# Jason9339/Wavelet-Noise-in-ray-tracing

Hardware: AMD Instinct MI355X
Metric: Mnoise-samples/sec (3D wavelet, octave=4) (higher is better)
Workload: dtype f32; 1 GPU; 512^3 dense 3D WNoise grid, tile=128, octave=4 (configs[1]); tile=128, seed=12345, octave=4, device=AMD Radeon Graphics (gfx950:sramecc+:xnack-)

## Files before the change

wavelet-noise-in-ray-tracing_amd/csrc/wn_wavelet_multiband.hip:

```cpp
#include "wn_internal.hpp"

#include <algorithm>
#include <cmath>
#include <type_traits>

namespace {

using wn::GridArgs;

typedef float v4f __attribute__((ext_vector_type(4)));
typedef float v2f __attribute__((ext_vector_type(2)));

constexpr int kMaxNB = 5;
constexpr int kWW = 8, kPW = 4, kSW = 4;
constexpr int kWaves = kWW + kPW + kSW;
constexpr int kPasses = 2 * kPW;
constexpr int kBX = 512, kBY = 8, kBZ = 8;
constexpr int kRing = 4;
constexpr int kSlotZ = 8, kSlotX = 16;
constexpr int kMaxK = 5;
constexpr int kRRow = kPasses * 64;
constexpr int kRPlane = kBY * kRRow;
constexpr int kRingFloats = kRing * kBY * kBX;
constexpr int kBoxFloats = 6144;
constexpr int kDmaPlanes = kMaxNB;
constexpr int kDmaLanded = kBZ - 2;

struct MbBand {
    float oscale;
    float factor;
    int first_pass;
    int K;
    int box_off;
    int rowlen;
};

struct MbArgs {
    const float *coef;
    float *out;
    int n, nmask;
    GridArgs g;
    float inv_den;
    int nbx, nby, nbz;
    int all_full;
    MbBand band[kMaxNB];
    int pass_band[kPasses];
};

__device__ __forceinline__ float readlane_f(float v, int l)
{
    return __int_as_float(__builtin_amdgcn_readlane(__float_as_int(v), l));
}

template <int NB>
__global__ __launch_bounds__(64 * kWaves) void grid3d_mbp_kernel(const MbArgs a)
{
    extern __shared__ __attribute__((aligned(16))) float lds[];
    __shared__ __attribute__((aligned(16))) float s_box[kBoxFloats];
    __shared__ int s_mid[3][NB][32];
    __shared__ float s_w[3][NB][kSlotX][3];
    __shared__ float s_oscale[NB];
    __shared__ __attribute__((aligned(16))) float s_wy[NB][kMaxK][kBY];
    __shared__ float s_wz[NB][64];
    __shared__ int s_prep[NB][4];
    __shared__ int s_bandc[NB][4];

    const int tid = threadIdx.x, lane = tid & 63;
    const int wave = __builtin_amdgcn_readfirstlane(tid >> 6);
    const bool is_window = wave < kWW, is_collapse = wave >= kWW && wave < kWW + kPW;
    const GridArgs &g = a.g;
    float *const ring = lds + 2 * kRPlane;

    const int nyz = a.nby * a.nbz;
    const long long total = (long long)a.nbx * nyz;
    const int item0 = (int)(total * blockIdx.x / gridDim.x), item1 = (int)(total * (blockIdx.x + 1) / gridDim.x);
    const int nb = item1 - item0;
    if (nb <= 0) return;
    const int G = nb * kBZ;

    struct Brick { int bx, by, bz; };
    auto brick_of = [&](int item) {
        Brick k;
        k.bx = item / nyz;
        k.by = (item - k.bx * nyz) / a.nbz;
        k.bz = item - k.bx * nyz - k.by * a.nbz;
        return k;
    };
    auto advance = [&](Brick &k) {
        if (++k.bz == a.nbz) { k.bz = 0; ++k.by; }
        if (k.by == a.nby) { k.by = 0; ++k.bx; }
    };

    auto fill_tables = [&](int buf, const Brick &k) {
        int tt = tid;
        asm volatile("" : "+v"(tt));
        const int b = tt >> 5, slot = tt & 31;
        if (b < NB && slot < kSlotX + 2) {
            int idx;
            if (slot < kSlotZ) idx = min(k.by * kBY + slot, g.ny - 1);
            else if (slot < kSlotX) idx = g.z0 + min(k.bz * kBZ + slot - kSlotZ, g.nz - 1);
            else idx = (slot == kSlotX) ? k.bx * kBX : min(k.bx * kBX + kBX - 1, g.nx - 1);
            const float c = wn::lattice_coord_fast(idx, (float)g.den, a.inv_den, g.base_range, s_oscale[b], g.post_scale);
            int m;
            float w0, w1, w2;
            wn::bspline(c, m, w0, w1, w2);
            s_mid[buf][b][slot] = m;
            if (slot < kSlotX) {
                s_w[buf][b][slot][0] = w0;
                s_w[buf][b][slot][1] = w1;
                s_w[buf][b][slot][2] = w2;
            }
        }
    };
    auto sgpr = [](int v) { return __builtin_amdgcn_readfirstlane(v); };
    auto fresh_rows = [&](int b, int K, int tA, int tB, bool same_column) {
        const int d = sgpr(s_mid[tB][b][kSlotZ]) - sgpr(s_mid[tA][b][kSlotZ]);
        return (same_column && d >= 0 && d <= 2) ? d : K;
    };

    auto derive_tables = [&](int b, int tA, int tB, bool same_column, bool first) {
        const int l = lane;
        {
            const int K = s_bandc[b][0];
            const int kz0 = s_mid[tB][b][kSlotZ] - 1;
            const int kzm = (K == 4) ? (kz0 & 3) : ((kz0 + 20 * 65536) % 5);
            {
                const int zi = l >> 3, j = l & 7;
                int t0 = kzm + (s_mid[tB][b][kSlotZ + zi] - s_mid[tB][b][kSlotZ]);
                t0 -= (t0 >= K) ? K : 0;
                const float w0 = s_w[tB][b][kSlotZ + zi][0], w1 = s_w[tB][b][kSlotZ + zi][1], w2 = s_w[tB][b][kSlotZ + zi][2];
                s_wz[b][l] = j == 0 ? w0 : j == 1 ? w1 : j == 2 ? w2 : __int_as_float(t0);
            }
            if (l < kMaxK * kBY) {
                const int j = l >> 3, yi = l & 7;
                const int dd = j - (s_mid[tB][b][yi] - s_mid[tB][b][0]);
                const float w0 = s_w[tB][b][yi][0], w1 = s_w[tB][b][yi][1], w2 = s_w[tB][b][yi][2];
                float f = a.band[0].factor;
#pragma unroll
                for (int bb = 1; bb < NB; ++bb) f = (b == bb) ? a.band[bb].factor : f;
                s_wy[b][j][yi] = ((unsigned)dd <= 2u ? (dd == 0 ? w0 : dd == 1 ? w1 : w2) : 0.0f) * f;
            }
            if (l == 0) {
                const int dz = s_mid[tB][b][kSlotZ] - s_mid[tA][b][kSlotZ];
                s_prep[b][0] = kzm;
                s_prep[b][1] = (!first && same_column && dz >= 0 && dz <= 2) ? dz : K;
                s_prep[b][2] = (s_mid[tB][b][kSlotX] - 1) & 3;
            }
        }
    };

    Brick cur = brick_of(item0), nxt = cur;
    advance(nxt);
    Brick nxt2 = nxt;
    advance(nxt2);
    if (tid < NB) {
        int K = a.band[0].K, box_off = a.band[0].box_off, rowlen = a.band[0].rowlen, fp = a.band[0].first_pass;
#pragma unroll
        for (int bb = 1; bb < NB; ++bb) {
            K = (tid == bb) ? a.band[bb].K : K;
            box_off = (tid == bb) ? a.band[bb].box_off : box_off;
            rowlen = (tid == bb) ? a.band[bb].rowlen : rowlen;
            fp = (tid == bb) ? a.band[bb].first_pass : fp;
        }
        s_bandc[tid][0] = K;
        s_bandc[tid][1] = box_off;
        s_bandc[tid][2] = rowlen;
        s_bandc[tid][3] = fp;
        float os = a.band[0].oscale;
#pragma unroll
        for (int bb = 1; bb < NB; ++bb) os = (tid == bb) ? a.band[bb].oscale : os;
        s_oscale[tid] = os;
    }
    __syncthreads();
    fill_tables(0, cur);
    if (nb > 1) fill_tables(1, nxt);
    __syncthreads();
    int tb = 0, t = 0;
    auto next_brick = [&]() {
        cur = nxt;
        nxt = nxt2;
        advance(nxt2);
        tb = (tb == 2) ? 0 : tb + 1;
        ++t;
    };

    if (is_collapse) {
        struct Pass {
            int id, band, col0, box_off, rowlen;
            float factor;
        };
        Pass ps[2];
        int pk[2];
#pragma unroll
        for (int i = 0; i < 2; ++i) {
            Pass &P = ps[i];
            P.id = (wave - kWW) + kPW * i;
            P.band = sgpr(a.pass_band[P.id]);
            const int bb0 = max(P.band, 0);
            pk[i] = P.band >= 0 ? sgpr(s_bandc[bb0][0]) : 0;
            P.box_off = sgpr(s_bandc[bb0][1]);
            P.rowlen = sgpr(s_bandc[bb0][2]);
            P.col0 = 64 * (P.id - sgpr(s_bandc[bb0][3]));
            float f = a.band[0].factor;
#pragma unroll
            for (int bb = 1; bb < NB; ++bb) f = (bb0 == bb) ? a.band[bb].factor : f;
            P.factor = __int_as_float(sgpr(__float_as_int(f)));
        }
        auto prep_brick = [&](const Pass &P, auto &yc, float &wzv, auto kc) {
            constexpr int K = decltype(kc)::value;
            if constexpr (K > 0) {
                const int kzm = sgpr(s_prep[P.band][0]), d = sgpr(s_prep[P.band][1]);
                wzv = s_wz[P.band][lane];
                const float *img = s_box + P.box_off + min(sgpr(s_prep[P.band][2]) + P.col0 + lane, P.rowlen - 1);
#pragma unroll
                for (int sl = 0; sl < K; ++sl) {
                    const int tau = (sl - kzm + K) % K;
                    if (tau >= K - d) {
                        const float *row = img + (tau - (K - d)) * K * P.rowlen;
#pragma unroll
                        for (int j = 0; j < K; ++j) {
                            const float cj = row[j * P.rowlen];
                            const v2f c2 = {cj, cj};
#pragma unroll
                            for (int h = 0; h < 2; ++h) {
                                const v4f w4 = *reinterpret_cast<const v4f *>(&s_wy[P.band][j][4 * h]);
                                const v2f wlo = {w4.x, w4.y}, whi = {w4.z, w4.w};
                                yc[2 * h][sl] = (j == 0) ? wlo * c2 : __builtin_elementwise_fma(wlo, c2, yc[2 * h][sl]);
                                yc[2 * h + 1][sl] = (j == 0) ? whi * c2 : __builtin_elementwise_fma(whi, c2, yc[2 * h + 1][sl]);
                            }
                        }
                    }
                }
            }
        };
        auto p1_slice = [&](float *Rw, int zi, const auto &yc, float wzv, auto kc) {
            constexpr int K = decltype(kc)::value;
            if constexpr (K > 0) {
                const float w0 = readlane_f(wzv, zi * 8), w1 = readlane_f(wzv, zi * 8 + 1), w2 = readlane_f(wzv, zi * 8 + 2);
                const int t0 = __builtin_amdgcn_readlane(__float_as_int(wzv), zi * 8 + 3);
                auto taps = [&](auto tc) {
                    constexpr int T0 = decltype(tc)::value, T1 = (T0 + 1) % K, T2 = (T0 + 2) % K;
#pragma unroll
                    for (int p2 = 0; p2 < kBY / 2; ++p2) {
                        v2f v = v2f{w0, w0} * yc[p2][T0];
                        v = __builtin_elementwise_fma(v2f{w1, w1}, yc[p2][T1], v);
                        v = __builtin_elementwise_fma(v2f{w2, w2}, yc[p2][T2], v);
                        Rw[(2 * p2) * kRRow] = v.x;
                        Rw[(2 * p2 + 1) * kRRow] = v.y;
                    }
                };
                using std::integral_constant;
                if (t0 == 0) taps(integral_constant<int, 0>{});
                else if (t0 == 1) taps(integral_constant<int, 1>{});
                else if (t0 == 2) taps(integral_constant<int, 2>{});
                else if (t0 == 3 || K == 4) taps(integral_constant<int, 3>{});
                else taps(integral_constant<int, K - 1>{});
            }
        };
        auto collapse_role = [&](auto k0c, auto k1c) {
            constexpr int K0 = decltype(k0c)::value, K1 = decltype(k1c)::value;
            v2f yc0[kBY / 2][K0 > 0 ? K0 : 1], yc1[kBY / 2][K1 > 0 ? K1 : 1];
            float wzv0 = 0.0f, wzv1 = 0.0f;
            float *const Rw0 = lds + 64 * ps[0].id + lane, *const Rw1 = lds + 64 * ps[1].id + lane;
            wn::lds_barrier();
            prep_brick(ps[0], yc0, wzv0, k0c);
            prep_brick(ps[1], yc1, wzv1, k1c);
            p1_slice(Rw0, 0, yc0, wzv0, k0c);
            p1_slice(Rw1, 0, yc1, wzv1, k1c);
            wn::lds_barrier();
            for (int gp = 0; gp < G + 2; ++gp) {
                const int zi = gp & (kBZ - 1);
                if (gp < G) {
                    if (gp + 1 < G) {
                        if (zi == kBZ - 1) {
                            prep_brick(ps[0], yc0, wzv0, k0c);
                            prep_brick(ps[1], yc1, wzv1, k1c);
                        }
                        const int rs = ((gp + 1) & 1) * kRPlane;
                        p1_slice(Rw0 + rs, (gp + 1) & (kBZ - 1), yc0, wzv0, k0c);
                        p1_slice(Rw1 + rs, (gp + 1) & (kBZ - 1), yc1, wzv1, k1c);
                    }
                    if (zi == kBZ - 1) next_brick();
                }
                wn::lds_barrier();
            }
        };
        using std::integral_constant;
        const int k0 = pk[0], k1 = pk[1];
        if (k0 == 4 && k1 == 4) collapse_role(integral_constant<int, 4>{}, integral_constant<int, 4>{});
        else if (k0 == 4 && k1 == 5) collapse_role(integral_constant<int, 4>{}, integral_constant<int, 5>{});
        else if (k0 == 5 && k1 == 4) collapse_role(integral_constant<int, 5>{}, integral_constant<int, 4>{});
        else if (k0 == 5 && k1 == 5) collapse_role(integral_constant<int, 5>{}, integral_constant<int, 5>{});
        else if (k0 == 4) collapse_role(integral_constant<int, 4>{}, integral_constant<int, 0>{});
        else if (k0 == 5) collapse_role(integral_constant<int, 5>{}, integral_constant<int, 0>{});
        else collapse_role(integral_constant<int, 0>{}, integral_constant<int, 0>{});
    } else if (is_window) {
        const int xw = (wave >> 2) & 1, wr = wave & 3;
        float ww[NB][4][4];
        int wbase[NB];
        auto x_weights = [&](int tbuf, int bx) {
            const float den = (float)g.den;
            const int x0 = bx * kBX + xw * 256 + lane * 4;
            float xbase[4];
#pragma unroll
            for (int q = 0; q < 4; ++q) {
                const float xi = (float)min(x0 + q, g.nx - 1);
                xbase[q] = ((a.inv_den != 0.0f) ? xi * a.inv_den : xi / den) * g.base_range;
            }
#pragma unroll
            for (int b = 0; b < NB; ++b) {
                int m[4];
                float w[4][3];
#pragma unroll
                for (int q = 0; q < 4; ++q) {
                    float cc = xbase[q] * a.band[b].oscale;
                    cc = cc * g.post_scale;
                    wn::bspline(cc, m[q], w[q][0], w[q][1], w[q][2]);
                }
                wbase[b] = 64 * a.band[b].first_pass + m[0] - s_mid[tbuf][b][kSlotX];
#pragma unroll
                for (int q = 0; q < 4; ++q) {
                    const bool up = m[q] != m[0];
                    ww[b][q][0] = up ? 0.0f : w[q][0];
                    ww[b][q][1] = up ? w[q][0] : w[q][1];
                    ww[b][q][2] = up ? w[q][1] : w[q][2];
                    ww[b][q][3] = up ? w[q][2] : 0.0f;
                }
            }
        };
        auto phaseC = [&](int rslot, int ringslot) {
            float acc[2][4];
            const float *Rp = lds + rslot * kRPlane + wr * kRRow;
#pragma unroll
            for (int b = 0; b < NB; ++b) {
                float v[2][4];
#pragma unroll
                for (int h = 0; h < 2; ++h)
#pragma unroll
                    for (int i = 0; i < 4; ++i) v[h][i] = Rp[h * 4 * kRRow + wbase[b] + i];
#pragma unroll
                for (int h = 0; h < 2; ++h)
#pragma unroll
                    for (int q = 0; q < 4; ++q) {
                        float s = (b == 0) ? ww[b][q][0] * v[h][0] : __builtin_fmaf(ww[b][q][0], v[h][0], acc[h][q]);
                        s = __builtin_fmaf(ww[b][q][1], v[h][1], s);
                        s = __builtin_fmaf(ww[b][q][2], v[h][2], s);
                        s = __builtin_fmaf(ww[b][q][3], v[h][3], s);
                        acc[h][q] = s;
                    }
            }
#pragma unroll
            for (int h = 0; h < 2; ++h)
                *reinterpret_cast<v4f *>(ring + (ringslot * kBY + wr + 4 * h) * kBX + xw * 256 + lane * 4) =
                    v4f{acc[h][0], acc[h][1], acc[h][2], acc[h][3]};
        };

        x_weights(0, cur.bx);
        wn::lds_barrier();
        wn::lds_barrier();
        for (int gp = 0; gp < G + 2; ++gp) {
            const int zi = gp & (kBZ - 1);
            if (gp < G) {
                phaseC(gp & 1, gp & (kRing - 1));
                if (zi == kBZ - 1) {
                    const int tb1 = (tb == 2) ? 0 : tb + 1, tb2 = (tb1 == 2) ? 0 : tb1 + 1;
                    if (t + 2 < nb) fill_tables(tb2, nxt2);
                    if (t + 1 < nb && nxt.bx != cur.bx) x_weights(tb1, nxt.bx);
                    next_brick();
                }
            }
            wn::lds_barrier();
        }
    } else {
        const int sw = wave - (kWW + kPW);
        int bK[NB], bBox[NB], bRow[NB];
#pragma unroll
        for (int b = 0; b < NB; ++b) {
            bK[b] = sgpr(s_bandc[b][0]);
            bBox[b] = sgpr(s_bandc[b][1]);
            bRow[b] = sgpr(s_bandc[b][2]);
        }
        auto request_band = [&](auto bc, int tA, int tB, bool same_column, bool first) {
            constexpr int b = decltype(bc)::value;
            if constexpr (b < NB) {
                const int K = bK[b];
                const int d = first ? K : fresh_rows(b, K, tA, tB, same_column);
                const int jy0 = sgpr(s_mid[tB][b][0]) - 1, kz0 = sgpr(s_mid[tB][b][kSlotZ]) - 1 + (K - d);
                const int r = min(lane, K * K - 1);
                const int f = (K == 4) ? (r >> 2) : ((r * 13) >> 6);
                const int j = r - f * K;
                const int rowoff = (((kz0 + f) & a.nmask) * a.n + ((jy0 + j) & a.nmask)) * a.n;
                const int ix0 = (sgpr(s_mid[tB][b][kSlotX]) - 1) & ~3;
                const unsigned voff = (unsigned)((ix0 + 4 * lane) & a.nmask) * 4u;
                for (int rr = sw; rr < d * K; rr += kSW) {
                    const char *rowp = reinterpret_cast<const char *>(a.coef + __builtin_amdgcn_readlane(rowoff, rr));
                    if (4 * lane < bRow[b])
                        __builtin_amdgcn_global_load_lds((const __attribute__((address_space(1))) void *)(rowp + voff),
                                                         (__attribute__((address_space(3))) void *)&s_box[bBox[b] + rr * bRow[b]],
                                                         16, 0, 0);
                }
            }
        };
        Brick sb = cur;
        const size_t plane_stride = (size_t)g.ny * g.nx;
        float *orow = nullptr;
        auto brick_pointer = [&]() {
            orow = a.out + ((size_t)(sb.bz * kBZ) * g.ny + sb.by * kBY + 2 * sw) * g.nx + sb.bx * kBX + lane * 4;
        };
        brick_pointer();
        auto store_plane = [&](int p) {
            const int zi = p & (kBZ - 1), ringslot = p & (kRing - 1);
            const float *src = ring + (ringslot * kBY + 2 * sw) * kBX + lane * 4;
            v4f v[4];
#pragma unroll
            for (int q = 0; q < 4; ++q) v[q] = *reinterpret_cast<const v4f *>(src + (q >> 1) * kBX + (q & 1) * 256);
            if (a.all_full) {
#pragma unroll
                for (int q = 0; q < 4; ++q) *reinterpret_cast<v4f *>(orow + (size_t)(q >> 1) * g.nx + (q & 1) * 256) = v[q];
            } else {
                const int z = sb.bz * kBZ + zi;
#pragma unroll
                for (int q = 0; q < 4; ++q) {
                    const int row = 2 * sw + (q >> 1), xh = q & 1;
                    const int y = sb.by * kBY + row, x = sb.bx * kBX + xh * 256 + lane * 4;
                    if (y < g.ny && z < g.nz && x + 3 < g.nx)
                        *reinterpret_cast<v4f *>(orow + (size_t)(q >> 1) * g.nx + (q & 1) * 256) = v[q];
                }
            }
            orow += plane_stride;
            if (zi == kBZ - 1) {
                advance(sb);
                brick_pointer();
            }
        };

        using std::integral_constant;
        request_band(integral_constant<int, 0>{}, 0, 0, false, true);
        request_band(integral_constant<int, 1>{}, 0, 0, false, true);
        request_band(integral_constant<int, 2>{}, 0, 0, false, true);
        request_band(integral_constant<int, 3>{}, 0, 0, false, true);
        request_band(integral_constant<int, 4>{}, 0, 0, false, true);
        for (int b = sw; b < NB; b += kSW) derive_tables(b, 0, 0, false, true);
        asm volatile("s_waitcnt vmcnt(0)" ::: "memory");
        wn::lds_barrier();
        wn::lds_barrier();
        for (int gp = 0; gp < G + 2; ++gp) {
            const int zi = gp & (kBZ - 1);
            if (gp >= 2) store_plane(gp - 2);
            if (gp < G) {
                if (zi < NB && t + 1 < nb) {
                    const int tb1 = (tb == 2) ? 0 : tb + 1;
                    const bool same = nxt.bx == cur.bx && nxt.by == cur.by;
                    if (zi == 0) request_band(integral_constant<int, 0>{}, tb, tb1, same, false);
                    else if (zi == 1) request_band(integral_constant<int, 1>{}, tb, tb1, same, false);
                    else if (zi == 2) request_band(integral_constant<int, 2>{}, tb, tb1, same, false);
                    else if (zi == 3) request_band(integral_constant<int, 3>{}, tb, tb1, same, false);
                    else request_band(integral_constant<int, 4>{}, tb, tb1, same, false);
                }
                if (zi == kBZ - 2 && t + 1 < nb)
                    for (int b = sw; b < NB; b += kSW)
                        derive_tables(b, tb, (tb == 2) ? 0 : tb + 1, nxt.bx == cur.bx && nxt.by == cur.by, false);
                if (zi == kDmaLanded) {
                    if (a.all_full) asm volatile("s_waitcnt vmcnt(%0)" ::"n"(4 * (kDmaLanded - kDmaPlanes + 1)) : "memory");
                    else asm volatile("s_waitcnt vmcnt(0)" ::: "memory");
                }
                if (zi == kBZ - 1) next_brick();
            }
            wn::lds_barrier();
        }
    }
}

template <int NB>
bool launch_mbp(const MbArgs &a, size_t lds, long long bricks, hipStream_t s)
{
    const void *fn = reinterpret_cast<const void *>(&grid3d_mbp_kernel<NB>);
    if (!wn::ensure_dynamic_lds(fn, wn::current_device(), lds)) return false;
    const int cus = wn::device_compute_units(wn::current_device());
    const int grid = (int)std::min<long long>(bricks, cus);
    hipLaunchKernelGGL((grid3d_mbp_kernel<NB>), dim3(grid), dim3(64 * kWaves), lds, s, a);
    return true;
}

}

namespace wn {

int multiband_try(const wn_tile *tile, const GridArgs &g, int nbands, const float *oscale, const float *weights,
                  float out_div, float *out_dev, hipStream_t stream, int min_bricks_per_cu)
{
    if (nbands < 1 || nbands > kMaxNB || tile->n == 0 || wn::pow2_mask(tile->n) < 0) return kDeclined;
    if (g.nx <= 256 || !vec4_ok(out_dev, g.nx) || g.ny <= 0 || g.nz <= 0 || g.z_const_mode || g.z0 < 0) return kDeclined;
    MbArgs a{};
    int passes = 0, box_off = 0;
    for (int w = 0; w < kPasses; ++w) a.pass_band[w] = -1;
    for (int b = 0; b < nbands; ++b) {
        LatticeStep ls;
        if (!lattice_step(g, oscale[b], false, false, 0.0, &ls) || !ls.two_mids()) return kDeclined;
        const int K = (int)std::max<long long>(4, std::max(ls.extent(kBY), ls.extent(kBZ)));
        if (K > kMaxK) return kDeclined;
        const int ex = (int)ls.extent(kBX) + 1;
        const int np = (ex + 63) / 64;
        if (passes + np > kPasses) return kDeclined;
        a.band[b].first_pass = passes;
        for (int p = 0; p < np; ++p) a.pass_band[passes++] = b;
        a.band[b].oscale = oscale[b];
        a.band[b].factor = (float)((double)(weights ? weights[b] : 1.0f) * (double)g.out_scale / (double)out_div);
        a.band[b].K = K;
        a.band[b].rowlen = (ex + 3 + 3) & ~3;
        if (a.band[b].rowlen > 256) return kDeclined;
        a.band[b].box_off = box_off;
        box_off += K * K * a.band[b].rowlen;
    }
    if (box_off > kBoxFloats) return kDeclined;
    const size_t lds = (size_t)(2 * kRPlane + kRingFloats) * sizeof(float);
    a.coef = tile->dev;
    a.out = out_dev;
    a.n = tile->n;
    a.nmask = wn::pow2_mask(tile->n);
    a.g = g;
    a.inv_den = wn::inv_den_of(g.den);
    a.nbx = (g.nx + kBX - 1) / kBX;
    a.nby = (g.ny + kBY - 1) / kBY;
    a.nbz = (g.nz + kBZ - 1) / kBZ;
    a.all_full = (g.nx % kBX == 0 && g.ny % kBY == 0 && g.nz % kBZ == 0) ? 1 : 0;
    const long long bricks = (long long)a.nbx * a.nby * a.nbz;
    if (bricks > 0x7fffffffLL / kBZ) return kDeclined;
    if (bricks < (long long)min_bricks_per_cu * wn::device_compute_units(wn::current_device())) return kDeclined;
    if ((long long)a.nbx * kBX * 10 > (long long)g.nx * 11) return kDeclined;
    bool ok;
    switch (nbands) {
    case 1: ok = launch_mbp<1>(a, lds, bricks, stream); break;
    case 2: ok = launch_mbp<2>(a, lds, bricks, stream); break;
    case 3: ok = launch_mbp<3>(a, lds, bricks, stream); break;
    case 4: ok = launch_mbp<4>(a, lds, bricks, stream); break;
    default: ok = launch_mbp<5>(a, lds, bricks, stream); break;
    }
    if (!ok) return kDeclined;
    WN_LAUNCH_CHECK("grid3d_mbp_kernel");
    return WN_OK;
}

}
```

Before: 1.419 million Msamples/s.

## Overlap prologue coefficient DMA with table fill and trim derive_tables work

The store waves now compute the first brick's lattice midpoints themselves and issue the initial coefficient row DMAs right away, while the other waves fill both table buffers in parallel. This replaces the two __syncthreads and the serialized first request_band calls. derive_tables now handles two bands per wave across lane halves with a compact z-weight layout, and recomputes the y-weight table only when the brick column changes. This mainly shortens per-block prologue latency and per-brick derive cost, at the price of more intricate lane mapping and duplicated midpoint computation.

```diff
diff --git a/wavelet-noise-in-ray-tracing_amd/csrc/wn_wavelet_multiband.hip b/wavelet-noise-in-ray-tracing_amd/csrc/wn_wavelet_multiband.hip
--- a/wavelet-noise-in-ray-tracing_amd/csrc/wn_wavelet_multiband.hip
+++ b/wavelet-noise-in-ray-tracing_amd/csrc/wn_wavelet_multiband.hip
@@ -91,16 +91,24 @@
         if (k.by == a.nby) { k.by = 0; ++k.bx; }
     };
 
-    auto fill_tables = [&](int buf, const Brick &k) {
-        int tt = tid;
+    auto oscale_of = [&](int b) {
+        float os = a.band[0].oscale;
+#pragma unroll
+        for (int bb = 1; bb < NB; ++bb) os = (b == bb) ? a.band[bb].oscale : os;
+        return os;
+    };
+    auto fill_tables = [&](int buf, const Brick &k, int tt, auto from_args) {
         asm volatile("" : "+v"(tt));
         const int b = tt >> 5, slot = tt & 31;
-        if (b < NB && slot < kSlotX + 2) {
+        if (tt >= 0 && b < NB && slot < kSlotX + 2) {
             int idx;
             if (slot < kSlotZ) idx = min(k.by * kBY + slot, g.ny - 1);
             else if (slot < kSlotX) idx = g.z0 + min(k.bz * kBZ + slot - kSlotZ, g.nz - 1);
             else idx = (slot == kSlotX) ? k.bx * kBX : min(k.bx * kBX + kBX - 1, g.nx - 1);
-            const float c = wn::lattice_coord_fast(idx, (float)g.den, a.inv_den, g.base_range, s_oscale[b], g.post_scale);
+            float os;
+            if constexpr (decltype(from_args)::value) os = oscale_of(b);
+            else os = s_oscale[b];
+            const float c = wn::lattice_coord_fast(idx, (float)g.den, a.inv_den, g.base_range, os, g.post_scale);
             int m;
             float w0, w1, w2;
             wn::bspline(c, m, w0, w1, w2);
@@ -118,34 +126,40 @@
         return (same_column && d >= 0 && d <= 2) ? d : K;
     };
 
-    auto derive_tables = [&](int b, int tA, int tB, bool same_column, bool first) {
+    auto derive_tables = [&](int sw, int tA, int tB, bool same_column, bool first) {
         const int l = lane;
         {
-            const int K = s_bandc[b][0];
-            const int kz0 = s_mid[tB][b][kSlotZ] - 1;
-            const int kzm = (K == 4) ? (kz0 & 3) : ((kz0 + 20 * 65536) % 5);
-            {
-                const int zi = l >> 3, j = l & 7;
-                int t0 = kzm + (s_mid[tB][b][kSlotZ + zi] - s_mid[tB][b][kSlotZ]);
-                t0 -= (t0 >= K) ? K : 0;
-                const float w0 = s_w[tB][b][kSlotZ + zi][0], w1 = s_w[tB][b][kSlotZ + zi][1], w2 = s_w[tB][b][kSlotZ + zi][2];
-                s_wz[b][l] = j == 0 ? w0 : j == 1 ? w1 : j == 2 ? w2 : __int_as_float(t0);
-            }
-            if (l < kMaxK * kBY) {
-                const int j = l >> 3, yi = l & 7;
-                const int dd = j - (s_mid[tB][b][yi] - s_mid[tB][b][0]);
-                const float w0 = s_w[tB][b][yi][0], w1 = s_w[tB][b][yi][1], w2 = s_w[tB][b][yi][2];
-                float f = a.band[0].factor;
-#pragma unroll
-                for (int bb = 1; bb < NB; ++bb) f = (b == bb) ? a.band[bb].factor : f;
-                s_wy[b][j][yi] = ((unsigned)dd <= 2u ? (dd == 0 ? w0 : dd == 1 ? w1 : w2) : 0.0f) * f;
-            }
-            if (l == 0) {
-                const int dz = s_mid[tB][b][kSlotZ] - s_mid[tA][b][kSlotZ];
-                s_prep[b][0] = kzm;
-                s_prep[b][1] = (!first && same_column && dz >= 0 && dz <= 2) ? dz : K;
-                s_prep[b][2] = (s_mid[tB][b][kSlotX] - 1) & 3;
-            }
+            const int b = sw + kSW * (l >> 5), q = l & 31;
+            if (b < NB) {
+                const int K = s_bandc[b][0];
+                const int kz0 = s_mid[tB][b][kSlotZ] - 1;
+                const int kzm = (K == 4) ? (kz0 & 3) : ((kz0 + 20 * 65536) % 5);
+                {
+                    const int zi = q >> 2, j = q & 3;
+                    int t0 = kzm + (s_mid[tB][b][kSlotZ + zi] - s_mid[tB][b][kSlotZ]);
+                    t0 -= (t0 >= K) ? K : 0;
+                    const float w0 = s_w[tB][b][kSlotZ + zi][0], w1 = s_w[tB][b][kSlotZ + zi][1], w2 = s_w[tB][b][kSlotZ + zi][2];
+                    s_wz[b][zi * 8 + j] = j == 0 ? w0 : j == 1 ? w1 : j == 2 ? w2 : __int_as_float(t0);
+                }
+                if (q == 0) {
+                    const int dz = s_mid[tB][b][kSlotZ] - s_mid[tA][b][kSlotZ];
+                    s_prep[b][0] = kzm;
+                    s_prep[b][1] = (!first && same_column && dz >= 0 && dz <= 2) ? dz : K;
+                    s_prep[b][2] = (s_mid[tB][b][kSlotX] - 1) & 3;
+                }
+            }
+        }
+        if (first || !same_column) {
+            for (int b = sw; b < NB; b += kSW)
+                if (l < kMaxK * kBY) {
+                    const int j = l >> 3, yi = l & 7;
+                    const int dd = j - (s_mid[tB][b][yi] - s_mid[tB][b][0]);
+                    const float w0 = s_w[tB][b][yi][0], w1 = s_w[tB][b][yi][1], w2 = s_w[tB][b][yi][2];
+                    float f = a.band[0].factor;
+#pragma unroll
+                    for (int bb = 1; bb < NB; ++bb) f = (b == bb) ? a.band[bb].factor : f;
+                    s_wy[b][j][yi] = ((unsigned)dd <= 2u ? (dd == 0 ? w0 : dd == 1 ? w1 : w2) : 0.0f) * f;
+                }
         }
     };
 
@@ -171,10 +185,38 @@
         for (int bb = 1; bb < NB; ++bb) os = (tid == bb) ? a.band[bb].oscale : os;
         s_oscale[tid] = os;
     }
-    __syncthreads();
-    fill_tables(0, cur);
-    if (nb > 1) fill_tables(1, nxt);
-    __syncthreads();
+    auto request_rows = [&](int sw, int K, int box, int rowlen, int d, int my, int mz, int mx) {
+        const int jy0 = my - 1, kz0 = mz - 1 + (K - d);
+        const int r = min(lane, K * K - 1);
+        const int f = (K == 4) ? (r >> 2) : ((r * 13) >> 6);
+        const int j = r - f * K;
+        const int rowoff = (((kz0 + f) & a.nmask) * a.n + ((jy0 + j) & a.nmask)) * a.n;
+        const int ix0 = (mx - 1) & ~3;
+        const unsigned voff = (unsigned)((ix0 + 4 * lane) & a.nmask) * 4u;
+        for (int rr = sw; rr < d * K; rr += kSW) {
+            const char *rowp = reinterpret_cast<const char *>(a.coef + __builtin_amdgcn_readlane(rowoff, rr));
+            if (4 * lane < rowlen)
+                __builtin_amdgcn_global_load_lds((const __attribute__((address_space(1))) void *)(rowp + voff),
+                                                 (__attribute__((address_space(3))) void *)&s_box[box + rr * rowlen], 16, 0, 0);
+        }
+    };
+    if (wave >= kWW + kPW) {
+        const int b = lane >> 2, which = lane & 3;
+        const int idx = which == 0 ? min(cur.by * kBY, g.ny - 1) : which == 1 ? g.z0 + min(cur.bz * kBZ, g.nz - 1) : cur.bx * kBX;
+        const float c = wn::lattice_coord_fast(idx, (float)g.den, a.inv_den, g.base_range, oscale_of(b), g.post_scale);
+        int m;
+        float w0, w1, w2;
+        wn::bspline(c, m, w0, w1, w2);
+#pragma unroll
+        for (int bb = 0; bb < NB; ++bb)
+            request_rows(wave - (kWW + kPW), a.band[bb].K, a.band[bb].box_off, a.band[bb].rowlen, a.band[bb].K,
+                         __builtin_amdgcn_readlane(m, 4 * bb), __builtin_amdgcn_readlane(m, 4 * bb + 1),
+                         __builtin_amdgcn_readlane(m, 4 * bb + 2));
+    } else {
+        fill_tables(0, cur, tid, std::true_type{});
+        if (nb > 1) fill_tables(1, nxt, tid - 192, std::true_type{});
+    }
+    wn::lds_barrier();
     int tb = 0, t = 0;
     auto next_brick = [&]() {
         cur = nxt;
@@ -364,7 +406,7 @@
                 phaseC(gp & 1, gp & (kRing - 1));
                 if (zi == kBZ - 1) {
                     const int tb1 = (tb == 2) ? 0 : tb + 1, tb2 = (tb1 == 2) ? 0 : tb1 + 1;
-                    if (t + 2 < nb) fill_tables(tb2, nxt2);
+                    if (t + 2 < nb) fill_tables(tb2, nxt2, tid, std::false_type{});
                     if (t + 1 < nb && nxt.bx != cur.bx) x_weights(tb1, nxt.bx);
                     next_brick();
                 }
@@ -380,26 +422,11 @@
             bBox[b] = sgpr(s_bandc[b][1]);
             bRow[b] = sgpr(s_bandc[b][2]);
         }
-        auto request_band = [&](auto bc, int tA, int tB, bool same_column, bool first) {
+        auto request_band = [&](auto bc, int tA, int tB, bool same_column) {
             constexpr int b = decltype(bc)::value;
-            if constexpr (b < NB) {
-                const int K = bK[b];
-                const int d = first ? K : fresh_rows(b, K, tA, tB, same_column);
-                const int jy0 = sgpr(s_mid[tB][b][0]) - 1, kz0 = sgpr(s_mid[tB][b][kSlotZ]) - 1 + (K - d);
-                const int r = min(lane, K * K - 1);
-                const int f = (K == 4) ? (r >> 2) : ((r * 13) >> 6);
-                const int j = r - f * K;
-                const int rowoff = (((kz0 + f) & a.nmask) * a.n + ((jy0 + j) & a.nmask)) * a.n;
-                const int ix0 = (sgpr(s_mid[tB][b][kSlotX]) - 1) & ~3;
-                const unsigned voff = (unsigned)((ix0 + 4 * lane) & a.nmask) * 4u;
-                for (int rr = sw; rr < d * K; rr += kSW) {
-                    const char *rowp = reinterpret_cast<const char *>(a.coef + __builtin_amdgcn_readlane(rowoff, rr));
-                    if (4 * lane < bRow[b])
-                        __builtin_amdgcn_global_load_lds((const __attribute__((address_space(1))) void *)(rowp + voff),
-                                                         (__attribute__((address_space(3))) void *)&s_box[bBox[b] + rr * bRow[b]],
-                                                         16, 0, 0);
-                }
-            }
+            if constexpr (b < NB)
+                request_rows(sw, bK[b], bBox[b], bRow[b], fresh_rows(b, bK[b], tA, tB, same_column), sgpr(s_mid[tB][b][0]),
+                             sgpr(s_mid[tB][b][kSlotZ]), sgpr(s_mid[tB][b][kSlotX]));
         };
         Brick sb = cur;
         const size_t plane_stride = (size_t)g.ny * g.nx;
@@ -435,12 +462,7 @@
         };
 
         using std::integral_constant;
-        request_band(integral_constant<int, 0>{}, 0, 0, false, true);
-        request_band(integral_constant<int, 1>{}, 0, 0, false, true);
-        request_band(integral_constant<int, 2>{}, 0, 0, false, true);
-        request_band(integral_constant<int, 3>{}, 0, 0, false, true);
-        request_band(integral_constant<int, 4>{}, 0, 0, false, true);
-        for (int b = sw; b < NB; b += kSW) derive_tables(b, 0, 0, false, true);
+        derive_tables(sw, 0, 0, false, true);
         asm volatile("s_waitcnt vmcnt(0)" ::: "memory");
         wn::lds_barrier();
         wn::lds_barrier();
@@ -451,15 +473,14 @@
                 if (zi < NB && t + 1 < nb) {
                     const int tb1 = (tb == 2) ? 0 : tb + 1;
                     const bool same = nxt.bx == cur.bx && nxt.by == cur.by;
-                    if (zi == 0) request_band(integral_constant<int, 0>{}, tb, tb1, same, false);
-                    else if (zi == 1) request_band(integral_constant<int, 1>{}, tb, tb1, same, false);
-                    else if (zi == 2) request_band(integral_constant<int, 2>{}, tb, tb1, same, false);
-                    else if (zi == 3) request_band(integral_constant<int, 3>{}, tb, tb1, same, false);
-                    else request_band(integral_constant<int, 4>{}, tb, tb1, same, false);
+                    if (zi == 0) request_band(integral_constant<int, 0>{}, tb, tb1, same);
+                    else if (zi == 1) request_band(integral_constant<int, 1>{}, tb, tb1, same);
+                    else if (zi == 2) request_band(integral_constant<int, 2>{}, tb, tb1, same);
+                    else if (zi == 3) request_band(integral_constant<int, 3>{}, tb, tb1, same);
+                    else request_band(integral_constant<int, 4>{}, tb, tb1, same);
                 }
                 if (zi == kBZ - 2 && t + 1 < nb)
-                    for (int b = sw; b < NB; b += kSW)
-                        derive_tables(b, tb, (tb == 2) ? 0 : tb + 1, nxt.bx == cur.bx && nxt.by == cur.by, false);
+                    derive_tables(sw, tb, (tb == 2) ? 0 : tb + 1, nxt.bx == cur.bx && nxt.by == cur.by, false);
                 if (zi == kDmaLanded) {
                     if (a.all_full) asm volatile("s_waitcnt vmcnt(%0)" ::"n"(4 * (kDmaLanded - kDmaPlanes + 1)) : "memory");
                     else asm volatile("s_waitcnt vmcnt(0)" ::: "memory");
```

Result: no change. 1.417 million Msamples/s (-0.1%).
